# libxsmm/tpp-mlir

Hardware: AMD Instinct MI355X
Metric: GFLOP/s on BRGEMM 1024^3 fp32 br=16 (xsmm_brgemm_invoke) (higher is better)
Workload: dtype f32; 1 GPU; BRGEMM 1024x1024x1024 fp32, batch-reduce=16 (m=n=1024 k=64 lda=ldb=ldc=1024 stride_a=64 stride_b=65536 BETA_0), one independent problem per GPU; launch=invoke-loop, kernel=brgemm_f32_fast_lw<64x64,k2>

## Files before the change

tpp-mlir_amd/csrc/brgemm_f32_lw.hip:

```cpp
#include "brgemm_f32_lw_tile.h"
#include "chain_args.h"
#include "split_scratch.h"
#include <type_traits>

namespace tpp {

typedef __attribute__((address_space(1))) unsigned int g_u32_lw;

template <int WM, int WN, int WK, bool GROUPED, int NL = 1, int NSLOT = LW_NSLOT, int NLB = NL, bool SPLIT = false, bool TAIL = false>
__global__ __launch_bounds__(64 * (WM * WN * WK + NL + NLB)) void brgemm_f32_lw(GemmArgs p, const WorkItem *__restrict__ items) {
  static_assert(!TAIL || (!GROUPED && !SPLIT), "the tail split is an instance of its own");
  constexpr bool MAYSPLIT = SPLIT || TAIL;
  using Tile = LwTile<WM, WN, WK, NSLOT>;
  constexpr int NMW = Tile::NMW, BM = Tile::BM, BN = Tile::BN, IPG = Tile::IPG;

  const int tid = threadIdx.x, lane = tid & 63;
  const int hw_wave = __builtin_amdgcn_readfirstlane(tid >> 6);
  const int wave = hw_wave < NL + NLB ? NMW + hw_wave : hw_wave - (NL + NLB);
  static_assert(!SPLIT || WK > 1, "the split epilogue is the K-split tiles' float4 epilogue");
  constexpr bool RAGN = GROUPED || SPLIT;
  WorkItem it{p.A, p.B, p.C, p.D, (int64_t)p.br};
  int tm, tn, sp = 0, tile_id = 0;
  bool is_tail = false;
  if constexpr (TAIL) {
    const int per_block = p.tiles_m * p.tiles_n;
    const int xshift = (p.m / BM) * (p.n / BN) == per_block ? 0 : 3;
    const int body_per = p.tail_body >> xshift, tail_per = per_block - body_per;
    const int u = (int)blockIdx.x, x = u & ((1 << xshift) - 1);
    int lt = u >> xshift;
    is_tail = u >= p.tail_body;
    if (is_tail) {
      const int j = (u - p.tail_body) >> xshift, t = j % tail_per;
      sp = j / tail_per;
      tile_id = x * tail_per + t;
      lt = body_per + t;
    }
    const int tz = lt / p.tiles_n;
    tm = (x >> p.xn_shift) * p.tiles_m + tz;
    tn = (x & ((1 << p.xn_shift) - 1)) * p.tiles_n + (lt - tz * p.tiles_n);
  } else if constexpr (SPLIT && GROUPED) {
    const int item = (int)blockIdx.x / p.split;
    sp = (int)blockIdx.x - item * p.split;
    if (items) it = items[item];
    tm = (int)blockIdx.z, tn = (int)blockIdx.y;
    tile_id = (item * (int)gridDim.y + tn) * (int)gridDim.z + tm;
  } else if constexpr (SPLIT) {
    const int tiles = p.tiles_m * p.tiles_n, total = tiles * p.split;
    int u = (int)blockIdx.x;
    if ((total & 7) == 0) u = (u & 7) * (total >> 3) + (u >> 3);
    sp = u / tiles;
    tile_id = u - sp * tiles;
    tn = tile_id / p.tiles_m;
    tm = tile_id - tn * p.tiles_m;
  } else {
    if constexpr (GROUPED) {
      if (items) it = items[blockIdx.x];
    }
    tm = GROUPED ? (int)blockIdx.z : (int)(blockIdx.x >> p.xn_shift) * p.tiles_m + (int)blockIdx.z;
    tn = GROUPED ? (int)blockIdx.y : (int)(blockIdx.x & ((1u << p.xn_shift) - 1)) * p.tiles_n + (int)blockIdx.y;
  }
  const int m0 = tm * BM, n0 = tn * BN;
  const int nvalid = RAGN ? p.n - n0 : BN;
  const float *__restrict__ A = (const float *)it.A;
  const float *__restrict__ B = (const float *)it.B;
  float *__restrict__ C = (float *)it.C;
  const bool pair = GROUPED && p.k == 32;
  const int kchunks = pair ? 1 : p.k / LW_BK;
  const int Tall = pair ? (int)it.br / 2 : (int)it.br * kchunks;
  const int nsplit = TAIL && !is_tail ? 1 : p.split;
  const int t_first = MAYSPLIT ? (int)(((long long)Tall * sp) / nsplit) : 0;
  const int T = MAYSPLIT ? (int)(((long long)Tall * (sp + 1)) / nsplit) - t_first : Tall;

  if (wave >= NMW) {
    typename Tile::template Loader<NL, NLB> ld(wave - NMW, lane, A, B, m0, n0, (int)p.lda, (int)p.ldb, p.stride_a, p.stride_b, kchunks, pair, nvalid);
    if constexpr (MAYSPLIT) ld.start_at(t_first);
    lw_loader_schedule<NSLOT>(T, [&](int slot) __attribute__((always_inline)) { ld.issue(slot); },
                              [&](int chunks) __attribute__((always_inline)) { ld.wait_left(chunks); });
    return;
  }

  const typename Tile::Wave w(wave, lane);
  const int wk = w.wk, wm = w.wm, wn = w.wn;
  const int li = lane & 31, lh = lane >> 5;
  const int ccol = n0 + wn * 32 + li;
  const __amdgpu_buffer_rsrc_t rsrcC =
      __builtin_amdgcn_make_buffer_rsrc((void *)(C + (int64_t)m0 * p.ldc + n0), 0, 0x7fffffff, 0x00020000);
  const unsigned voffC = (unsigned)(((wm * 32 + 4 * lh) * (int)p.ldc + wn * 32 + li) * 4);
  const unsigned ldcb = (unsigned)((int)p.ldc * 4);
  f32x16 acc;
#pragma unroll
  for (int r = 0; r < 16; ++r) acc[r] = 0.0f;
  float bias = 0.0f;
  if constexpr (WK == 1) {
    if ((p.ep & EP_BIAS) && (!RAGN || ccol < p.n)) bias = ((const float *)it.D)[ccol];
  }
  constexpr bool BIAS_EARLY = WK > 1 && WM * WN * WK <= 4;
  f32x4 bias4 = {0.0f, 0.0f, 0.0f, 0.0f};
  const bool piece_ok = !RAGN || wn * 32 + 4 * (lane & 7) < nvalid;
  if constexpr (BIAS_EARLY) {
    if ((p.ep & EP_BIAS) && piece_ok) bias4 = *(const f32x4 *)((const float *)it.D + n0 + wn * 32 + 4 * (lane & 7));
  }
  if (wk == 0 && !SPLIT && !(TAIL && is_tail)) {
    if (!(p.ep & EP_BETA0) && (!RAGN || ccol < p.n)) {
#pragma unroll
      for (int r = 0; r < 16; ++r)
        acc[r] = __builtin_bit_cast(
            float, __builtin_amdgcn_raw_buffer_load_b32(rsrcC, voffC, (unsigned)((r & 3) + 8 * (r >> 2)) * ldcb, 0));
    }
  }

  __builtin_amdgcn_s_barrier();
  __builtin_amdgcn_sched_barrier(0);
  if (T > 0) Tile::mfma_chunks(acc, T, w);

  if constexpr (WK > 1) {
    Tile::park_partials(acc, w);
    if constexpr (!BIAS_EARLY) {
      if ((p.ep & EP_BIAS) && piece_ok) bias4 = *(const f32x4 *)((const float *)it.D + n0 + wn * 32 + 4 * (lane & 7));
    }
    f32x4 part[IPG];
    Tile::sum_partials(part, w);
    if (MAYSPLIT && (!TAIL || is_tail)) {
      constexpr int TILE = BM * BN;
      const int S = nsplit;
      float *scr = p.scratch + (size_t)tile_id * S * TILE;
      const __amdgpu_buffer_rsrc_t rsrcS = __builtin_amdgcn_make_buffer_rsrc((void *)scr, 0, 0x7fffffff, 0x00020000);
      const unsigned pvo = (unsigned)((wave * 64 + lane) * 16);
#pragma unroll
      for (int j = 0; j < IPG; ++j)
        __builtin_amdgcn_raw_buffer_store_b128(__builtin_bit_cast(u32x4, part[j]), rsrcS, pvo, (unsigned)((sp * TILE + j * NMW * 256) * 4), 16);
      asm volatile("s_waitcnt vmcnt(0)" ::: "memory");
      __syncthreads();
      unsigned *flag = (unsigned *)smem_lw;
      if (wave == 0 && lane == 0)
        *flag = __hip_atomic_fetch_add((g_u32_lw *)(p.split_cnt + tile_id), 1u, __ATOMIC_RELAXED, __HIP_MEMORY_SCOPE_AGENT);
      __syncthreads();
      if (*flag != (unsigned)(S - 1)) return;
      if (wave == 0 && lane == 0) __hip_atomic_store((g_u32_lw *)(p.split_cnt + tile_id), 0u, __ATOMIC_RELAXED, __HIP_MEMORY_SCOPE_AGENT);
#pragma unroll
      for (int j = 0; j < IPG; ++j) {
        f32x4 acc4 = __builtin_bit_cast(f32x4, __builtin_amdgcn_raw_buffer_load_b128(rsrcS, pvo, (unsigned)((j * NMW * 256) * 4), 16));
        int s2 = 1;
        for (; s2 + 4 <= S; s2 += 4) {
          f32x4 t[4];
#pragma unroll
          for (int e = 0; e < 4; ++e)
            t[e] = __builtin_bit_cast(f32x4, __builtin_amdgcn_raw_buffer_load_b128(rsrcS, pvo, (unsigned)(((s2 + e) * TILE + j * NMW * 256) * 4), 16));
#pragma unroll
          for (int e = 0; e < 4; ++e) acc4 += t[e];
        }
        for (; s2 < S; ++s2)
          acc4 += __builtin_bit_cast(f32x4, __builtin_amdgcn_raw_buffer_load_b128(rsrcS, pvo, (unsigned)((s2 * TILE + j * NMW * 256) * 4), 16));
        part[j] = acc4;
      }
#pragma unroll
      for (int j = 0; j < IPG; ++j) {
        if (!(p.ep & EP_BETA0) && piece_ok) part[j] += __builtin_bit_cast(f32x4, __builtin_amdgcn_raw_buffer_load_b128(rsrcC, Tile::piece_off(w, j, (int)p.ldc), 0, 0));
      }
    }
    Tile::finish(part, bias4, p.ep, rsrcC, (int)p.ldc, piece_ok, w);
    return;
  }
#pragma unroll
  for (int r = 0; r < 16; ++r) {
    float v = acc[r] + bias;
    if (p.ep & EP_RELU) v = v > 0.0f ? v : 0.0f;
    if (!RAGN || ccol < p.n)
      __builtin_amdgcn_raw_buffer_store_b32(__builtin_bit_cast(unsigned, v), rsrcC, voffC,
                                            (unsigned)((r & 3) + 8 * (r >> 2)) * ldcb, LW_C_AUX);
  }
}

typedef __attribute__((address_space(1))) unsigned int g_u32_f32c;
template <int WM, int WN, int WK, int NL>
__global__ __launch_bounds__(64 * (WM * WN * WK + 2 * NL)) void brgemm_f32_lw_chain(ChainArgs p) {
  static_assert(WK > 1, "the hand-off needs the 16-byte stores of the K-split tiles' epilogue");
  using Tile = LwTile<WM, WN, WK>;
  constexpr int NMW = Tile::NMW, BM = Tile::BM, BN = Tile::BN;

  const int tid = threadIdx.x, lane = tid & 63;
  const int hw_wave = __builtin_amdgcn_readfirstlane(tid >> 6);
  const int wave = hw_wave < 2 * NL ? NMW + hw_wave : hw_wave - 2 * NL;
  const int tm = (int)blockIdx.x / p.tiles_n, tn = (int)blockIdx.x % p.tiles_n;
  const int m0 = tm * BM, n0 = tn * BN;
  const int L = p.nlayers;

  if (wave >= NMW) {
    const bool isA = (wave - NMW) < NL;
    for (int l = 0; l < L; ++l) {
      const ChainLayer &Y = p.L[l];
      const int lda = (int)(l == 0 ? p.lda : p.L[l > 0 ? l - 1 : 0].ldc);
      const float *Asrc = (const float *)(l == 0 ? p.A : p.L[l > 0 ? l - 1 : 0].C);
      const int kchunks = Y.k / LW_BK;
      typename Tile::template Loader<NL, NL> ld(wave - NMW, lane, Asrc, (const float *)Y.B, m0, n0, lda, (int)Y.ldb, Y.stride_a, Y.stride_b, kchunks, false, BN);
      const bool sc1 = isA && l > 0;
      if (sc1) {
        g_u32_f32c *c = (g_u32_f32c *)(p.cnt + ((size_t)(l - 1) * p.tiles_m + tm) * CHAIN_CNT_STRIDE);
        const unsigned target = p.target;
        const unsigned long long t0 = __builtin_amdgcn_s_memrealtime();
        for (;;) {
          const unsigned v = __hip_atomic_load(c, __ATOMIC_RELAXED, __HIP_MEMORY_SCOPE_AGENT);
          if ((int)(v - target) >= 0) break;
          if (__builtin_amdgcn_s_memrealtime() - t0 > CHAIN_TIMEOUT_TICKS) {
            if (lane == 0) __hip_atomic_store((g_u32_f32c *)p.err, 1u + (unsigned)l, __ATOMIC_RELAXED, __HIP_MEMORY_SCOPE_AGENT);
            break;
          }
          __builtin_amdgcn_s_sleep(1);
        }
        asm volatile("" ::: "memory");
      }
      lw_loader_schedule<LW_NSLOT>(Y.br * kchunks, [&](int slot) __attribute__((always_inline)) { ld.template issue<true>(slot, sc1); },
                                   [&](int chunks) __attribute__((always_inline)) { ld.wait_left(chunks); });
      __builtin_amdgcn_s_barrier();
      __builtin_amdgcn_s_barrier();
      if (l + 1 < L) __builtin_amdgcn_s_barrier();
    }
    return;
  }

  const typename Tile::Wave w(wave, lane);
  for (int l = 0; l < L; ++l) {
    const ChainLayer &Y = p.L[l];
    const int ldc = (int)Y.ldc;
    const __amdgpu_buffer_rsrc_t rsrcC = __builtin_amdgcn_make_buffer_rsrc((void *)((float *)Y.C + (int64_t)m0 * ldc + n0), 0, 0x7fffffff, 0x00020000);
    f32x16 acc;
#pragma unroll
    for (int r = 0; r < 16; ++r) acc[r] = 0.0f;
    __builtin_amdgcn_s_barrier();
    __builtin_amdgcn_sched_barrier(0);
    Tile::mfma_chunks(acc, Y.br * (Y.k / LW_BK), w);
    Tile::park_partials(acc, w);
    f32x4 bias4 = {0.0f, 0.0f, 0.0f, 0.0f}, part[Tile::IPG];
    if (Y.ep & EP_BIAS) bias4 = *(const f32x4 *)((const float *)Y.D + n0 + w.wn * 32 + 4 * (lane & 7));
    Tile::sum_partials(part, w);
    Tile::finish(part, bias4, Y.ep, rsrcC, ldc, true, w);
    if (l + 1 == L) break;
    asm volatile("s_waitcnt vmcnt(0) lgkmcnt(0)" ::: "memory");
    __builtin_amdgcn_s_barrier();
    if (wave == 0 && lane == 0)
      __hip_atomic_fetch_add((g_u32_f32c *)(p.cnt + ((size_t)l * p.tiles_m + tm) * CHAIN_CNT_STRIDE), 1u, __ATOMIC_RELAXED, __HIP_MEMORY_SCOPE_AGENT);
  }
}

template <int WM, int WN, int WK, int NL, int NSLOT, int NLB>
__global__ __launch_bounds__(64 * (WM * WN * WK + NL + NLB)) void brgemm_f32_lw_edge(GemmArgs p) {
  using Tile = LwTile<WM, WN, WK, NSLOT>;
  constexpr int NMW = Tile::NMW, BM = Tile::BM, BN = Tile::BN, IPG = Tile::IPG;

  const int tid = threadIdx.x, lane = tid & 63;
  const int hw_wave = __builtin_amdgcn_readfirstlane(tid >> 6);
  const int wave = hw_wave < NL + NLB ? NMW + hw_wave : hw_wave - (NL + NLB);
  const int tm = (int)(blockIdx.x >> p.xn_shift) * p.tiles_m + (int)blockIdx.z;
  const int tn = (int)(blockIdx.x & ((1u << p.xn_shift) - 1)) * p.tiles_n + (int)blockIdx.y;
  const int m0 = tm * BM < p.m - BM ? tm * BM : p.m - BM, n0 = tn * BN < p.n - BN ? tn * BN : p.n - BN;
  const int own_r = tm * BM - m0, own_c = tn * BN - n0;
  const float *__restrict__ A = (const float *)p.A;
  const float *__restrict__ B = (const float *)p.B;
  float *__restrict__ C = (float *)p.C;
  const int kchunks = p.k / LW_BK;
  const int T = p.br * kchunks;

  if (wave >= NMW) {
    typename Tile::template Loader<NL, NLB> ld(wave - NMW, lane, A, B, m0, n0, (int)p.lda, (int)p.ldb, p.stride_a, p.stride_b, kchunks, false, BN);
    lw_loader_schedule<NSLOT>(T, [&](int slot) __attribute__((always_inline)) { ld.issue(slot); },
                              [&](int chunks) __attribute__((always_inline)) { ld.wait_left(chunks); });
    return;
  }

  const typename Tile::Wave w(wave, lane);
  const int wk = w.wk, wm = w.wm, wn = w.wn;
  const int li = lane & 31, lh = lane >> 5;
  const __amdgpu_buffer_rsrc_t rsrcC =
      __builtin_amdgcn_make_buffer_rsrc((void *)(C + (int64_t)m0 * p.ldc + n0), 0, 0x7fffffff, 0x00020000);
  const unsigned voffC = (unsigned)(((wm * 32 + 4 * lh) * (int)p.ldc + wn * 32 + li) * 4);
  const unsigned ldcb = (unsigned)((int)p.ldc * 4);
  const bool col_owned = wn * 32 + li >= own_c;
  const int row_first = own_r - (wm * 32 + 4 * lh);
  f32x16 acc;
#pragma unroll
  for (int r = 0; r < 16; ++r) acc[r] = 0.0f;
  float bias = 0.0f;
  if constexpr (WK == 1) {
    if (p.ep & EP_BIAS) bias = ((const float *)p.D)[n0 + wn * 32 + li];
  }
  constexpr bool BIAS_EARLY = WK > 1 && WM * WN * WK <= 4;
  f32x4 bias4 = {0.0f, 0.0f, 0.0f, 0.0f};
  if constexpr (BIAS_EARLY) {
    if (p.ep & EP_BIAS) bias4 = *(const f32x4 *)((const float *)p.D + n0 + wn * 32 + 4 * (lane & 7));
  }
  if (wk == 0 && !(p.ep & EP_BETA0) && col_owned) {
#pragma unroll
    for (int r = 0; r < 16; ++r)
      if ((r & 3) + 8 * (r >> 2) >= row_first)
        acc[r] = __builtin_bit_cast(float, __builtin_amdgcn_raw_buffer_load_b32(rsrcC, voffC, (unsigned)((r & 3) + 8 * (r >> 2)) * ldcb, 0));
  }

  __builtin_amdgcn_s_barrier();
  __builtin_amdgcn_sched_barrier(0);
  if (T > 0) Tile::mfma_chunks(acc, T, w);

  if constexpr (WK > 1) {
    Tile::park_partials(acc, w);
    if constexpr (!BIAS_EARLY) {
      if (p.ep & EP_BIAS) bias4 = *(const f32x4 *)((const float *)p.D + n0 + wn * 32 + 4 * (lane & 7));
    }
    f32x4 part[IPG];
    Tile::sum_partials(part, w);
    Tile::finish_owned(part, bias4, p.ep, rsrcC, (int)p.ldc, own_r, own_c, w);
    return;
  }
#pragma unroll
  for (int r = 0; r < 16; ++r) {
    float v = acc[r] + bias;
    if (p.ep & EP_RELU) v = v > 0.0f ? v : 0.0f;
    if (col_owned && (r & 3) + 8 * (r >> 2) >= row_first)
      __builtin_amdgcn_raw_buffer_store_b32(__builtin_bit_cast(unsigned, v), rsrcC, voffC, (unsigned)((r & 3) + 8 * (r >> 2)) * ldcb, LW_C_AUX);
  }
}

template <int WM, int WN, int WK, int NL, int NSLOT, int NLB>
__global__ __launch_bounds__(64 * (WM * WN * WK + NL + NLB)) void brgemm_f32_lw_kedge(GemmArgs p) {
  using Tile = LwTile<WM, WN, WK, NSLOT>;
  constexpr int NMW = Tile::NMW, BM = Tile::BM, BN = Tile::BN, IPG = Tile::IPG;

  const int tid = threadIdx.x, lane = tid & 63;
  const int hw_wave = __builtin_amdgcn_readfirstlane(tid >> 6);
  const int wave = hw_wave < NL + NLB ? NMW + hw_wave : hw_wave - (NL + NLB);
  const int tm = (int)(blockIdx.x >> p.xn_shift) * p.tiles_m + (int)blockIdx.z;
  const int tn = (int)(blockIdx.x & ((1u << p.xn_shift) - 1)) * p.tiles_n + (int)blockIdx.y;
  const int m0 = tm * BM < p.m - BM ? tm * BM : p.m - BM, n0 = tn * BN < p.n - BN ? tn * BN : p.n - BN;
  const int own_r = tm * BM - m0, own_c = tn * BN - n0;
  const float *__restrict__ A = (const float *)p.A;
  const float *__restrict__ B = (const float *)p.B;
  float *__restrict__ C = (float *)p.C;
  const int kchunks = kedge_chunks(p.k);
  const int T = p.br * kchunks;

  if (wave >= NMW) {
    typename Tile::template Loader<NL, NLB> ld(wave - NMW, lane, A, B, m0, n0, (int)p.lda, (int)p.ldb, p.stride_a, p.stride_b, kchunks, false, BN);
    ld.ragged_k(p.k);
    lw_loader_schedule<NSLOT>(T, [&](int slot) __attribute__((always_inline)) { ld.issue_ragged(slot); },
                              [&](int chunks) __attribute__((always_inline)) { ld.wait_left(chunks); });
    return;
  }

  const typename Tile::Wave w(wave, lane);
  const int wk = w.wk, wm = w.wm, wn = w.wn;
  const int li = lane & 31, lh = lane >> 5;
  const __amdgpu_buffer_rsrc_t rsrcC =
      __builtin_amdgcn_make_buffer_rsrc((void *)(C + (int64_t)m0 * p.ldc + n0), 0, 0x7fffffff, 0x00020000);
  const unsigned voffC = (unsigned)(((wm * 32 + 4 * lh) * (int)p.ldc + wn * 32 + li) * 4);
  const unsigned ldcb = (unsigned)((int)p.ldc * 4);
  const bool col_owned = wn * 32 + li >= own_c;
  const int row_first = own_r - (wm * 32 + 4 * lh);
  f32x16 acc;
#pragma unroll
  for (int r = 0; r < 16; ++r) acc[r] = 0.0f;
  float bias = 0.0f;
  if constexpr (WK == 1) {
    if (p.ep & EP_BIAS) bias = ((const float *)p.D)[n0 + wn * 32 + li];
  }
  constexpr bool BIAS_EARLY = WK > 1 && WM * WN * WK <= 4;
  f32x4 bias4 = {0.0f, 0.0f, 0.0f, 0.0f};
  if constexpr (BIAS_EARLY) {
    if (p.ep & EP_BIAS) bias4 = *(const f32x4 *)((const float *)p.D + n0 + wn * 32 + 4 * (lane & 7));
  }
  if (wk == 0 && !(p.ep & EP_BETA0) && col_owned) {
#pragma unroll
    for (int r = 0; r < 16; ++r)
      if ((r & 3) + 8 * (r >> 2) >= row_first)
        acc[r] = __builtin_bit_cast(float, __builtin_amdgcn_raw_buffer_load_b32(rsrcC, voffC, (unsigned)((r & 3) + 8 * (r >> 2)) * ldcb, 0));
  }

  __builtin_amdgcn_s_barrier();
  __builtin_amdgcn_sched_barrier(0);
  Tile::mfma_chunks_ragged(acc, T, kchunks, kedge_skip_blocks(p.k, kchunks - 1), w);

  if constexpr (WK > 1) {
    Tile::park_partials(acc, w);
    if constexpr (!BIAS_EARLY) {
      if (p.ep & EP_BIAS) bias4 = *(const f32x4 *)((const float *)p.D + n0 + wn * 32 + 4 * (lane & 7));
    }
    f32x4 part[IPG];
    Tile::sum_partials(part, w);
    Tile::finish_owned(part, bias4, p.ep, rsrcC, (int)p.ldc, own_r, own_c, w);
    return;
  }
#pragma unroll
  for (int r = 0; r < 16; ++r) {
    float v = acc[r] + bias;
    if (p.ep & EP_RELU) v = v > 0.0f ? v : 0.0f;
    if (col_owned && (r & 3) + 8 * (r >> 2) >= row_first)
      __builtin_amdgcn_raw_buffer_store_b32(__builtin_bit_cast(unsigned, v), rsrcC, voffC, (unsigned)((r & 3) + 8 * (r >> 2)) * ldcb, LW_C_AUX);
  }
}

static int lw_xcd_blocks(const GemmArgs &a, int tiles_m, int tiles_n) {
  int xm = 0;
  long long best = -1;
  for (int c : {4, 2, 8, 1}) {
    const int xn = 8 / c;
    if (tiles_m % c || tiles_n % xn || tiles_m / c > 65535 || tiles_n / xn > 65535) continue;
    const long long cost = (long long)a.m / c + (long long)a.n / xn;
    if (best < 0 || cost < best) {
      best = cost;
      xm = c;
    }
  }
  return xm;
}

static bool lw_xcd_grid(GemmArgs &args, int tiles_m, int tiles_n, bool allow_blocks = true) {
  const int xm = allow_blocks ? lw_xcd_blocks(args, tiles_m, tiles_n) : 0, xn = xm ? 8 / xm : 1;
  args.tiles_m = xm ? tiles_m / xm : tiles_m;
  args.tiles_n = tiles_n / xn;
  args.xn_shift = xn == 8 ? 3 : xn == 4 ? 2 : xn == 2 ? 1 : 0;
  return xm != 0;
}

static bool lw_split_scratch(GemmArgs &args, hipStream_t s, long long tiles, int S, int tile_floats) {
  const SplitScratch *sc = split_scratch_for(s, tiles, tiles * S * tile_floats);
  if (!sc) return false;
  args.split = S;
  args.scratch = sc->partial;
  args.split_cnt = sc->cnt;
  return true;
}

template <int WM, int WN, int WK, bool GROUPED = false, int NL = 1, int NSLOT = LW_NSLOT, int NLB = NL, bool SPLIT = false, bool TAIL = false> struct LwLayer {
  using Tile = LwTile<WM, WN, WK, NSLOT>;
  static constexpr int NT = 64 * (Tile::NMW + NL + NLB);
  static constexpr auto kernel = brgemm_f32_lw<WM, WN, WK, GROUPED, NL, NSLOT, NLB, SPLIT, TAIL>;
};
template <int WM, int WN, int WK, int NL> struct LwChain {
  using Tile = LwTile<WM, WN, WK>;
  static constexpr int NT = 64 * (Tile::NMW + 2 * NL);
  static constexpr auto kernel = brgemm_f32_lw_chain<WM, WN, WK, NL>;
};
template <int WM, int WN, int WK, int NL, int NSLOT, int NLB> struct LwEdge {
  using Tile = LwTile<WM, WN, WK, NSLOT>;
  static constexpr int NT = 64 * (Tile::NMW + NL + NLB);
  static constexpr auto kernel = brgemm_f32_lw_edge<WM, WN, WK, NL, NSLOT, NLB>;
};
template <int WM, int WN, int WK, int NL, int NSLOT, int NLB> struct LwKEdge {
  using Tile = LwTile<WM, WN, WK, NSLOT>;
  static constexpr int NT = 64 * (Tile::NMW + NL + NLB);
  static constexpr auto kernel = brgemm_f32_lw_kedge<WM, WN, WK, NL, NSLOT, NLB>;
};
template <class I, class... Args> static hipError_t lw_launch(dim3 grid, hipStream_t s, const Args &...args) {
  static std::atomic<unsigned long long> lds_set{0};
  if (hipError_t e = ensure_dynamic_lds((const void *)I::kernel, (int)I::Tile::LDS_BYTES, lds_set); e != hipSuccess) return e;
  hipLaunchKernelGGL(I::kernel, grid, dim3(I::NT), I::Tile::LDS_BYTES, s, args...);
  return hipGetLastError();
}

template <int WM, int WN, int WK, int NL = 1, int NSLOT = LW_NSLOT, int NLB = NL> static hipError_t launch_lw_t(const GemmArgs &a, hipStream_t s) {
  using I = LwLayer<WM, WN, WK, false, NL, NSLOT, NLB>;
  GemmArgs args = a;
  const bool blocks = lw_xcd_grid(args, a.m / I::Tile::BM, a.n / I::Tile::BN);
  if (args.tiles_m > 65535 || args.tiles_n > 65535) return hipErrorInvalidValue;
  return lw_launch<I>(dim3(blocks ? 8 : 1, args.tiles_n, args.tiles_m), s, args, (const WorkItem *)nullptr);
}

template <int WM, int WN, int WK, bool SPLIT>
static hipError_t launch_lw_grouped_t(const GemmArgs &a, const WorkItem *items, int n_items, int S, hipStream_t s) {
  using I = LwLayer<WM, WN, WK, true, 1, LW_NSLOT, 1, SPLIT>;
  constexpr int BM = I::Tile::BM, BN = I::Tile::BN;
  const int tiles_m = a.m / BM, tiles_n = (a.n + BN - 1) / BN;
  GemmArgs args = a;
  args.tiles_m = args.tiles_n = 0;
  args.xn_shift = 0;
  if (SPLIT && !lw_split_scratch(args, s, (long long)n_items * tiles_m * tiles_n, S, BM * BN)) return hipErrorOutOfMemory;
  return lw_launch<I>(dim3((unsigned)(n_items * (SPLIT ? S : 1)), tiles_n, tiles_m), s, args, items);
}

template <int WM, int WN, int WK> static hipError_t launch_lw_split_t(const GemmArgs &a, int S, hipStream_t s) {
  using I = LwLayer<WM, WN, WK, false, 1, LW_NSLOT, 1, true>;
  constexpr int BM = I::Tile::BM, BN = I::Tile::BN;
  GemmArgs args = a;
  args.tiles_m = a.m / BM;
  args.tiles_n = (a.n + BN - 1) / BN;
  args.xn_shift = 0;
  const long long tiles = (long long)args.tiles_m * args.tiles_n;
  if (!lw_split_scratch(args, s, tiles, S, BM * BN)) return hipErrorOutOfMemory;
  return lw_launch<I>(dim3((unsigned)(tiles * S)), s, args, (const WorkItem *)nullptr);
}
template <int WM, int WN, int WK, int NL, int NLB> static hipError_t launch_lw_tail_t(const GemmArgs &a, int tail_tiles, int S, hipStream_t s) {
  using I = LwLayer<WM, WN, WK, false, NL, LW_NSLOT, NLB, false, true>;
  constexpr int BM = I::Tile::BM, BN = I::Tile::BN;
  const int tiles_m = a.m / BM, tiles_n = a.n / BN;
  const long long tiles = (long long)tiles_m * tiles_n, body = tiles - tail_tiles;
  if (a.m % BM || a.n % BN || tail_tiles <= 0 || body <= 0 || S < 2 || S > SPLIT_MAX || body + (long long)tail_tiles * S > 0x7fffffffLL)
    return hipErrorInvalidValue;
  GemmArgs args = a;
  if (!lw_split_scratch(args, s, tail_tiles, S, BM * BN)) return hipErrorOutOfMemory;
  lw_xcd_grid(args, tiles_m, tiles_n, body % 8 == 0 && tail_tiles % 8 == 0);
  args.tail_body = (int)body;
  return lw_launch<I>(dim3((unsigned)(body + (long long)tail_tiles * S)), s, args, (const WorkItem *)nullptr);
}

template <int WM, int WN, int WK, int NL = 1, int NSLOT = LW_NSLOT, int NLB = NL> static hipError_t launch_lw_edge_t(const GemmArgs &a, hipStream_t s) {
  using I = LwEdge<WM, WN, WK, NL, NSLOT, NLB>;
  constexpr int BM = I::Tile::BM, BN = I::Tile::BN;
  if (a.m < BM || a.n < BN || (a.n & 3) || a.k <= 0 || a.k % LW_BK || a.br < 1) return hipErrorInvalidValue;
  GemmArgs args = a;
  const bool blocks = lw_xcd_grid(args, (a.m + BM - 1) / BM, (a.n + BN - 1) / BN);
  if (args.tiles_m > 65535 || args.tiles_n > 65535) return hipErrorInvalidValue;
  return lw_launch<I>(dim3(blocks ? 8 : 1, args.tiles_n, args.tiles_m), s, args);
}

template <int WM, int WN, int WK, int NL = 1, int NSLOT = LW_NSLOT, int NLB = NL> static hipError_t launch_lw_kedge_t(const GemmArgs &a, hipStream_t s) {
  using I = LwKEdge<WM, WN, WK, NL, NSLOT, NLB>;
  constexpr int BM = I::Tile::BM, BN = I::Tile::BN;
  if (a.m < BM || a.n < BN || (a.n & 3) || !kedge_k_ok(a.k) || a.br < 1) return hipErrorInvalidValue;
  GemmArgs args = a;
  const bool blocks = lw_xcd_grid(args, (a.m + BM - 1) / BM, (a.n + BN - 1) / BN);
  if (args.tiles_m > 65535 || args.tiles_n > 65535) return hipErrorInvalidValue;
  return lw_launch<I>(dim3(blocks ? 8 : 1, args.tiles_n, args.tiles_m), s, args);
}

hipError_t launch_f32_lw_halves(const GemmArgs &a, hipStream_t s) {
  if (a.m <= 0 || a.n <= 0 || a.m % 64 || a.n % 64 || a.k <= 0 || a.k % LW_BK || a.br < 0) return hipErrorInvalidValue;
  return launch_lw_t<2, 1, 2, 2, 3, 1>(a, s);
}

hipError_t launch_f32_lw_grouped(int tile, const GemmArgs &a, const WorkItem *items, int n_items, int split, hipStream_t s) {
  if (split > 1) {
    hipError_t e = hipErrorInvalidValue;
    switch (tile) {
    case 1: e = launch_lw_grouped_t<2, 2, 2, true>(a, items, n_items, split, s); break;
    case 2: e = launch_lw_grouped_t<2, 1, 4, true>(a, items, n_items, split, s); break;
    case 3: e = launch_lw_grouped_t<1, 1, 4, true>(a, items, n_items, split, s); break;
    default: break;
    }
    if (e != hipErrorOutOfMemory && e != hipErrorInvalidValue) return e;
    (void)hipGetLastError();
  }
  switch (tile) {
  case 0: return launch_lw_grouped_t<2, 2, 1, false>(a, items, n_items, 1, s);
  case 1: return launch_lw_grouped_t<2, 2, 2, false>(a, items, n_items, 1, s);
  case 2: return launch_lw_grouped_t<2, 1, 4, false>(a, items, n_items, 1, s);
  case 3: return launch_lw_grouped_t<1, 1, 4, false>(a, items, n_items, 1, s);
  default: return hipErrorInvalidValue;
  }
}
hipError_t launch_f32_lw_split(int tile, const GemmArgs &a, int split, hipStream_t s) {
  switch (tile) {
  case 1: return launch_lw_split_t<2, 2, 2>(a, split, s);
  case 2: return launch_lw_split_t<2, 1, 4>(a, split, s);
  case 3: return launch_lw_split_t<1, 1, 4>(a, split, s);
  default: return hipErrorInvalidValue;
  }
}

hipError_t launch_f32_lw_tail(int tile, const GemmArgs &a, int tail_tiles, int split, hipStream_t s) {
  switch (tile) {
  case 1: return launch_lw_tail_t<2, 2, 2, 2, 2>(a, tail_tiles, split, s);
  case 2: return launch_lw_tail_t<2, 1, 4, 2, 1>(a, tail_tiles, split, s);
  case 3: return launch_lw_tail_t<1, 1, 4, 1, 1>(a, tail_tiles, split, s);
  default: return hipErrorInvalidValue;
  }
}

hipError_t launch_f32_lw_edge(int tile, const GemmArgs &a, hipStream_t s) {
  switch (tile) {
  case 1: return launch_lw_edge_t<2, 2, 2, 2>(a, s);
  case 2: return launch_lw_edge_t<2, 1, 4, 2, LW_NSLOT, 1>(a, s);
  case 3: return launch_lw_edge_t<1, 1, 4>(a, s);
  case 4: return launch_lw_edge_t<4, 2, 1, 2, 3>(a, s);
  default: return hipErrorInvalidValue;
  }
}

hipError_t launch_f32_lw_kedge(int tile, const GemmArgs &a, hipStream_t s) {
  switch (tile) {
  case 1: return launch_lw_kedge_t<2, 2, 2, 2>(a, s);
  case 2: return launch_lw_kedge_t<2, 1, 4, 2, LW_NSLOT, 1>(a, s);
  case 3: return launch_lw_kedge_t<1, 1, 4>(a, s);
  case 4: return launch_lw_kedge_t<4, 2, 1, 2, 3>(a, s);
  default: return hipErrorInvalidValue;
  }
}

template <int WM, int WN, int WK, int NL> static hipError_t launch_f32_chain_t(const ChainArgs &a, hipStream_t s) {
  using I = LwChain<WM, WN, WK, NL>;
  ChainArgs args = a;
  args.tiles_m = a.m / I::Tile::BM;
  args.tiles_n = a.n / I::Tile::BN;
  const long long tiles = (long long)args.tiles_m * args.tiles_n;
  if (tiles <= 0 || tiles > 0x7fffffffLL) return hipErrorInvalidValue;
  return lw_launch<I>(dim3((unsigned)tiles), s, args);
}

hipError_t launch_f32_chain(int tile, const ChainArgs &a, hipStream_t s) {
  switch (tile) {
  case 1: return launch_f32_chain_t<2, 2, 2, 2>(a, s);
  case 2: return launch_f32_chain_t<2, 1, 4, 1>(a, s);
  default: return hipErrorInvalidValue;
  }
}

hipError_t launch_f32_lw(int tile, const GemmArgs &a, hipStream_t s) {
  switch (tile) {
  case 0: return launch_lw_t<2, 2, 1>(a, s);
  case 1: return launch_lw_t<2, 2, 2, 2>(a, s);
  case 2: return launch_lw_t<2, 1, 4, 2, LW_NSLOT, 1>(a, s);
  case 3: return launch_lw_t<1, 1, 4>(a, s);
  case 4: return launch_lw_t<4, 2, 1, 2, 3>(a, s);
  default: return hipErrorInvalidValue;
  }
}

}
```

tpp-mlir_amd/csrc/brgemm_f32_lw_tile.h:

```cpp
#pragma once
#include "brgemm_f32_lw_kedge.h"
#include "gemm_common.h"
#include "xsmm_desc.h"
#include <type_traits>

namespace tpp {

constexpr int LW_BK = 64;
constexpr int LW_NSLOT = 4;
constexpr int LW_C_AUX = C_STORE_AUX;
static_assert(KEDGE_BK == LW_BK, "the ragged-k schedule is written for this chunk");

typedef __attribute__((address_space(3))) void lds_void_lw;
extern __shared__ __attribute__((aligned(16))) float smem_lw[];

template <int NSLOT, class Issue, class Wait> __device__ __forceinline__ void lw_loader_schedule(int T, Issue &&issue, Wait &&wait_left) {
  if (T > 0) issue(0);
  if (T > 1) issue(1);
  wait_left(T > 1 ? 1 : 0);
  __builtin_amdgcn_s_barrier();
  if (NSLOT > 3 && T > 2) issue(2);
  for (int t = 0; t + 1 < T; ++t) {
    wait_left(NSLOT > 3 && t + 2 < T ? 1 : 0);
    __builtin_amdgcn_s_barrier();
    if (t + NSLOT - 1 < T) issue((t + NSLOT - 1) % NSLOT);
  }
}

template <int WM, int WN, int WK, int NSLOT = LW_NSLOT> struct LwTile {
  static constexpr int NMW = WM * WN * WK;
  static constexpr int BM = 32 * WM, BN = 32 * WN;
  static constexpr int A_STAGE = BM * LW_BK, B_STAGE = LW_BK * BN, SLOT = A_STAGE + B_STAGE;
  static constexpr int NA = BM / 4;
  static constexpr int RPI = 256 / BN;
  static constexpr int NB = LW_BK / RPI;
  static constexpr int KB_PER_WAVE = 8 / WK, KB_HALF = KB_PER_WAVE / 2;
  static constexpr int IPG = WK > 1 ? 4 / WK : 1;
  static constexpr size_t LDS_BYTES = (size_t)NSLOT * SLOT * sizeof(float);
  static_assert(KB_HALF >= 1, "tile outside the schedule's limits");
  static_assert(NSLOT == 3 || NSLOT == 4, "ring depth");
  static_assert(LDS_BYTES <= 160 * 1024, "LDS budget");

  template <int NL, int NLB> struct Loader {
    static_assert(NA % NL == 0 && NB % NLB == 0, "panel instructions divide over the loader waves");
    static_assert(NA / NL <= 31 && NB / NLB <= 31, "tile outside the schedule's limits (vmcnt is 6 bits)");
    bool isA;
    int part, kc, kchunks;
    unsigned voA[4], voA2[2], voB, stepA, stepB, pairB;
    const float *g;
    int64_t d_in, d_batch, d_wrap;

    __device__ __forceinline__ Loader(int lw, int lane, const float *A, const float *B, int m0, int n0, int lda, int ldb, int64_t stride_a,
                                      int64_t stride_b, int kchunks_, bool pair, int nvalid)
        : isA(lw < NL), part(lw < NL ? lw : lw - NL), kc(0), kchunks(kchunks_) {
#pragma unroll
      for (int j = 0; j < 4; ++j) {
        const int r = 4 * j + (lane >> 4), pc = (lane & 15) ^ r;
        voA[j] = (unsigned)((r * lda + (pair ? (pc >> 3) * (int)stride_a + 4 * (pc & 7) : 4 * pc)) * 4);
      }
#pragma unroll
      for (int j = 0; j < 2; ++j) {
        const int r = 4 * (part + 2 * j) + (lane >> 4), pc = (lane & 15) ^ r;
        voA2[j] = (unsigned)((r * lda + (pair ? (pc >> 3) * (int)stride_a + 4 * (pc & 7) : 4 * pc)) * 4);
      }
      const int pieceB = nvalid < BN ? (lane % (BN / 4) < nvalid / 4 ? lane % (BN / 4) : nvalid / 4 - 1) : lane % (BN / 4);
      voB = (unsigned)(((lane / (BN / 4)) * ldb + 4 * pieceB) * 4);
      stepA = (unsigned)(16 * lda * 4), stepB = (unsigned)(RPI * ldb * 4);
      pairB = pair ? (unsigned)(((int)stride_b - 32 * ldb) * 4) : 0u;
      g = isA ? A + (int64_t)m0 * lda : B + n0;
      d_in = isA ? (int64_t)LW_BK : (int64_t)LW_BK * ldb;
      d_batch = (isA ? stride_a : stride_b) * (pair ? 2 : 1);
      d_wrap = d_batch - (int64_t)(kchunks - 1) * d_in;
    }
    __device__ __forceinline__ void start_at(int t_first) {
      const int b0 = t_first / kchunks;
      kc = t_first - b0 * kchunks;
      g += (int64_t)b0 * d_batch + (int64_t)kc * d_in;
    }
    template <int AUX> __device__ __forceinline__ void load_a(float *base, __amdgpu_buffer_rsrc_t r) const {
#pragma unroll
      for (int i = 0; i < NA / NL; ++i) {
        const int v = part + NL * i;
        __builtin_amdgcn_raw_ptr_buffer_load_lds(r, (lds_void_lw *)(base + v * 256), 16, NL == 1 ? voA[i & 3] : NL == 2 ? voA2[i & 1] : voA2[0],
                                                 (unsigned)(v >> 2) * stepA, 0, AUX);
      }
    }
    template <bool MAY_SC1 = false> __device__ __forceinline__ void issue(int slot, bool sc1 = false) {
      float *base = smem_lw + slot * SLOT + (isA ? 0 : A_STAGE);
      const __amdgpu_buffer_rsrc_t r = __builtin_amdgcn_make_buffer_rsrc((void *)g, 0, 0x7fffffff, 0x00020000);
      if (isA) {
        if (MAY_SC1 && sc1) load_a<16>(base, r);
        else load_a<0>(base, r);
      } else {
#pragma unroll
        for (int i = 0; i < NB / NLB; ++i) {
          const int v = part + NLB * i;
          __builtin_amdgcn_raw_ptr_buffer_load_lds(r, (lds_void_lw *)(base + v * 256), 16, voB, (unsigned)v * stepB + (v * RPI >= 32 ? pairB : 0u), 0, 0);
        }
      }
      if (++kc == kchunks) {
        kc = 0;
        g += d_wrap;
      } else {
        g += d_in;
      }
    }
    int64_t d_fix;
    __device__ __forceinline__ void ragged_k(int k) {
      const int64_t unit = d_in / LW_BK;
      d_fix = (int64_t)(kedge_step(k, kchunks - 2) - LW_BK) * unit;
      d_wrap = d_batch - (int64_t)kedge_chunk_start(k, kchunks - 1) * unit;
    }
    __device__ __forceinline__ void issue_ragged(int slot) {
      issue(slot);
      if (kc == kchunks - 1) g += d_fix;
    }
    __device__ __forceinline__ void wait_left(int chunks) const {
      if (chunks == 0) asm volatile("s_waitcnt vmcnt(0)" ::: "memory");
      else if (isA) asm volatile("s_waitcnt vmcnt(%0)" ::"n"(NA / NL) : "memory");
      else asm volatile("s_waitcnt vmcnt(%0)" ::"n"(NB / NLB) : "memory");
    }
  };

  struct Wave {
    int wk, wmn, wm, wn, lane;
    __device__ __forceinline__ Wave(int wave, int lane_) : wk(wave / (WM * WN)), wmn(wave % (WM * WN)), wm(wmn / WN), wn(wmn % WN), lane(lane_) {}
  };

  static __device__ __forceinline__ void mfma_chunks(f32x16 &acc, int T, const Wave &w) {
    f32x4 fa[2];
    float fb[2][4];
    const int li = w.lane & 31, lh = w.lane >> 5;
    const int a_off = (w.wm * 32 + li) * LW_BK, b_off = w.wn * 32 + li;
    auto frag_load = [&](int buf, int slot, int kb) __attribute__((always_inline)) {
      const float *as = smem_lw + slot * SLOT + a_off;
      const float *bs = smem_lw + slot * SLOT + A_STAGE + b_off;
      fa[buf] = *(const f32x4 *)(as + (((2 * kb + lh) ^ (li & 15)) << 2));
#pragma unroll
      for (int s = 0; s < 4; ++s) fb[buf][s] = bs[(8 * kb + 4 * lh + s) * BN];
    };
    const int kbw = w.wk * KB_PER_WAVE;
    auto chunk = [&](auto slot_c, auto hn_c, bool has_next_rt) __attribute__((always_inline)) {
      constexpr int S = decltype(slot_c)::value, NS = (S + 1) % NSLOT;
      const bool has_next = decltype(hn_c)::value == 1 ? true : has_next_rt;
#pragma unroll
      for (int q = 0; q < KB_PER_WAVE; ++q) {
        const int cur = q & 1, nxt = cur ^ 1;
        if (q + 1 < KB_PER_WAVE) frag_load(nxt, S, kbw + q + 1);
        else frag_load(nxt, NS, kbw);
        __builtin_amdgcn_sched_barrier(0);
#pragma unroll
        for (int s = 0; s < 4; ++s) acc = __builtin_amdgcn_mfma_f32_32x32x2f32(fa[cur][s], fb[cur][s], acc, 0, 0, 0);
        __builtin_amdgcn_sched_barrier(0);
        if (q == KB_HALF - 1 && has_next) {
          __builtin_amdgcn_s_barrier();
          __builtin_amdgcn_sched_barrier(0);
        }
      }
      constexpr int PF = KB_PER_WAVE & 1;
      if constexpr (decltype(hn_c)::value != 1)
        asm volatile("" : "+v"(fa[PF]), "+v"(fb[PF][0]), "+v"(fb[PF][1]), "+v"(fb[PF][2]), "+v"(fb[PF][3]));
    };
    using S0 = std::integral_constant<int, 0>;
    using S1 = std::integral_constant<int, 1>;
    using S2 = std::integral_constant<int, 2>;
    using S3 = std::integral_constant<int, 3>;
    using HY = std::integral_constant<int, 1>;
    using HR = std::integral_constant<int, 2>;

    frag_load(0, 0, kbw);
    int t = 0;
    for (; t + NSLOT < T; t += NSLOT) {
      chunk(S0{}, HY{}, true);
      chunk(S1{}, HY{}, true);
      chunk(S2{}, HY{}, true);
      if constexpr (NSLOT > 3) chunk(S3{}, HY{}, true);
    }
    for (;;) {
      chunk(S0{}, HR{}, t + 1 < T);
      if (++t == T) break;
      chunk(S1{}, HR{}, t + 1 < T);
      if (++t == T) break;
      chunk(S2{}, HR{}, t + 1 < T);
      if (++t == T) break;
      if constexpr (NSLOT > 3) {
        chunk(S3{}, HR{}, t + 1 < T);
        if (++t == T) break;
      }
    }
  }

  static __device__ __forceinline__ void mfma_chunks_ragged(f32x16 &acc, int T, int kchunks, int skip, const Wave &w) {
    f32x4 fa[2];
    float fb[2][4];
    const int li = w.lane & 31, lh = w.lane >> 5;
    const int a_off = (w.wm * 32 + li) * LW_BK, b_off = w.wn * 32 + li;
    auto frag_load = [&](int buf, int slot, int kb) __attribute__((always_inline)) {
      const float *as = smem_lw + slot * SLOT + a_off;
      const float *bs = smem_lw + slot * SLOT + A_STAGE + b_off;
      fa[buf] = *(const f32x4 *)(as + (((2 * kb + lh) ^ (li & 15)) << 2));
#pragma unroll
      for (int s = 0; s < 4; ++s) fb[buf][s] = bs[(8 * kb + 4 * lh + s) * BN];
    };
    const int kbw = w.wk * KB_PER_WAVE;
    auto chunk = [&](auto slot_c, auto rag_c, int first, bool has_next_rt) __attribute__((always_inline)) {
      constexpr int S = decltype(slot_c)::value, NS = (S + 1) % NSLOT;
      constexpr bool RAG = decltype(rag_c)::value != 0;
      const bool has_next = RAG ? has_next_rt : true;
#pragma unroll
      for (int q = 0; q < KB_PER_WAVE; ++q) {
        const int cur = q & 1, nxt = cur ^ 1;
        if (q + 1 < KB_PER_WAVE) frag_load(nxt, S, kbw + q + 1);
        else frag_load(nxt, NS, kbw);
        __builtin_amdgcn_sched_barrier(0);
        if (!RAG || kedge_block_runs(kbw + q, first)) {
#pragma unroll
          for (int s = 0; s < 4; ++s) acc = __builtin_amdgcn_mfma_f32_32x32x2f32(fa[cur][s], fb[cur][s], acc, 0, 0, 0);
        }
        __builtin_amdgcn_sched_barrier(0);
        if (q == KB_HALF - 1 && has_next) {
          __builtin_amdgcn_s_barrier();
          __builtin_amdgcn_sched_barrier(0);
        }
      }
      constexpr int PF = KB_PER_WAVE & 1;
      if constexpr (RAG) asm volatile("" : "+v"(fa[PF]), "+v"(fb[PF][0]), "+v"(fb[PF][1]), "+v"(fb[PF][2]), "+v"(fb[PF][3]));
    };
    using S0 = std::integral_constant<int, 0>;
    using S1 = std::integral_constant<int, 1>;
    using S2 = std::integral_constant<int, 2>;
    using S3 = std::integral_constant<int, 3>;
    using R0 = std::integral_constant<int, 0>;
    using R1 = std::integral_constant<int, 1>;

    frag_load(0, 0, kbw);
    int t = 0, c = 0;
    for (;;) {
      if (c + NSLOT < kchunks) {
        chunk(S0{}, R0{}, 0, true);
        chunk(S1{}, R0{}, 0, true);
        chunk(S2{}, R0{}, 0, true);
        if constexpr (NSLOT > 3) chunk(S3{}, R0{}, 0, true);
        t += NSLOT, c += NSLOT;
        continue;
      }
      chunk(S0{}, R1{}, c + 1 == kchunks ? skip : 0, t + 1 < T);
      if (++t == T) break;
      if (++c == kchunks) c = 0;
      chunk(S1{}, R1{}, c + 1 == kchunks ? skip : 0, t + 1 < T);
      if (++t == T) break;
      if (++c == kchunks) c = 0;
      chunk(S2{}, R1{}, c + 1 == kchunks ? skip : 0, t + 1 < T);
      if (++t == T) break;
      if (++c == kchunks) c = 0;
      if constexpr (NSLOT > 3) {
        chunk(S3{}, R1{}, c + 1 == kchunks ? skip : 0, t + 1 < T);
        if (++t == T) break;
        if (++c == kchunks) c = 0;
      }
    }
  }

  static __device__ __forceinline__ void park_partials(const f32x16 &acc, const Wave &w) {
    __syncthreads();
    float *dst = smem_lw + (w.wk * (WM * WN) + w.wmn) * 1024 + w.lane;
#pragma unroll
    for (int r = 0; r < 16; ++r) dst[r * 64] = acc[r];
    __syncthreads();
  }
  static __device__ __forceinline__ int piece_row(const Wave &w, int j) { return 8 * (w.wk * IPG + j) + (w.lane >> 3); }
  static __device__ __forceinline__ unsigned piece_off(const Wave &w, int j, int ldc) {
    return (unsigned)(((w.wm * 32 + piece_row(w, j)) * ldc + w.wn * 32 + 4 * (w.lane & 7)) * 4);
  }
  static __device__ __forceinline__ void sum_partials(f32x4 (&part)[IPG], const Wave &w) {
#pragma unroll
    for (int j = 0; j < IPG; ++j) {
      const int q = piece_row(w, j);
      const int r = (q & 3) + 4 * (q >> 3), lh2 = (q >> 2) & 1;
      const float *src = smem_lw + w.wmn * 1024 + r * 64 + lh2 * 32 + 4 * (w.lane & 7);
      f32x4 v = *(const f32x4 *)src;
#pragma unroll
      for (int g = 1; g < WK; ++g) v += *(const f32x4 *)(src + g * (WM * WN) * 1024);
      part[j] = v;
    }
  }
  static __device__ __forceinline__ void finish(const f32x4 (&part)[IPG], f32x4 bias4, int ep, __amdgpu_buffer_rsrc_t rsrcC, int ldc, bool ok, const Wave &w) {
#pragma unroll
    for (int j = 0; j < IPG; ++j) {
      f32x4 v = part[j] + bias4;
      if (ep & EP_RELU) {
#pragma unroll
        for (int e = 0; e < 4; ++e) v[e] = v[e] > 0.0f ? v[e] : 0.0f;
      }
      if (ok) __builtin_amdgcn_raw_buffer_store_b128(__builtin_bit_cast(u32x4, v), rsrcC, piece_off(w, j, ldc), 0, LW_C_AUX);
    }
  }
  static __device__ __forceinline__ bool piece_owned(const Wave &w, int j, int own_r, int own_c) {
    return w.wm * 32 + piece_row(w, j) >= own_r && w.wn * 32 + 4 * (w.lane & 7) >= own_c;
  }
  static __device__ __forceinline__ void finish_owned(const f32x4 (&part)[IPG], f32x4 bias4, int ep, __amdgpu_buffer_rsrc_t rsrcC, int ldc, int own_r, int own_c,
                                                      const Wave &w) {
#pragma unroll
    for (int j = 0; j < IPG; ++j) {
      f32x4 v = part[j] + bias4;
      if (ep & EP_RELU) {
#pragma unroll
        for (int e = 0; e < 4; ++e) v[e] = v[e] > 0.0f ? v[e] : 0.0f;
      }
      if (piece_owned(w, j, own_r, own_c)) __builtin_amdgcn_raw_buffer_store_b128(__builtin_bit_cast(u32x4, v), rsrcC, piece_off(w, j, ldc), 0, LW_C_AUX);
    }
  }
};

}
```

Before: 123,900 GFLOP/s.

## Precompute and pin LDS fragment and epilogue addresses; overlap loader setup with first load

Computes LDS fragment addresses, park/sum addresses and C store offsets once before the main loop and pins them in registers with empty asm constraints. This removes per-chunk address arithmetic from the MFMA loop. The loader now issues the first chunk's load before computing the batch/wrap strides, so setup work overlaps the first memory request. Kernel arguments are forced into scalar registers. The cost is higher VGPR pressure from holding the precomputed addresses, which could lower occupancy or cause spills.

Result: faster. 127,400 GFLOP/s, median of 6 (+2.8%).

```diff
diff --git a/tpp-mlir_amd/csrc/brgemm_f32_lw.hip b/tpp-mlir_amd/csrc/brgemm_f32_lw.hip
--- a/tpp-mlir_amd/csrc/brgemm_f32_lw.hip
+++ b/tpp-mlir_amd/csrc/brgemm_f32_lw.hip
@@ -61,8 +61,12 @@
   }
   const int m0 = tm * BM, n0 = tn * BN;
   const int nvalid = RAGN ? p.n - n0 : BN;
-  const float *__restrict__ A = (const float *)it.A;
-  const float *__restrict__ B = (const float *)it.B;
+  const float *A_ = (const float *)it.A, *B_ = (const float *)it.B;
+  int lda = (int)p.lda, ldb = (int)p.ldb;
+  int64_t stride_a = p.stride_a, stride_b = p.stride_b;
+  asm volatile("" : "+s"(A_), "+s"(B_), "+s"(lda), "+s"(ldb), "+s"(stride_a), "+s"(stride_b));
+  const float *__restrict__ A = A_;
+  const float *__restrict__ B = B_;
   float *__restrict__ C = (float *)it.C;
   const bool pair = GROUPED && p.k == 32;
   const int kchunks = pair ? 1 : p.k / LW_BK;
@@ -72,10 +76,17 @@
   const int T = MAYSPLIT ? (int)(((long long)Tall * (sp + 1)) / nsplit) - t_first : Tall;
 
   if (wave >= NMW) {
-    typename Tile::template Loader<NL, NLB> ld(wave - NMW, lane, A, B, m0, n0, (int)p.lda, (int)p.ldb, p.stride_a, p.stride_b, kchunks, pair, nvalid);
-    if constexpr (MAYSPLIT) ld.start_at(t_first);
+    typename Tile::template Loader<NL, NLB> ld(wave - NMW, lane, A, B, m0, n0, lda, ldb, stride_a, stride_b, kchunks, pair, nvalid);
+    if constexpr (MAYSPLIT) {
+      ld.finish_setup();
+      ld.start_at(t_first);
+    }
     lw_loader_schedule<NSLOT>(T, [&](int slot) __attribute__((always_inline)) { ld.issue(slot); },
-                              [&](int chunks) __attribute__((always_inline)) { ld.wait_left(chunks); });
+                              [&](int chunks) __attribute__((always_inline)) { ld.wait_left(chunks); },
+                              [&]() __attribute__((always_inline)) {
+                                if constexpr (MAYSPLIT) ld.issue(0);
+                                else ld.issue_first();
+                              });
     return;
   }
 
@@ -109,17 +120,21 @@
     }
   }
 
+  const auto fr = Tile::mfma_setup(w);
+  const auto tl = Tile::template tail_setup<!SPLIT>(w, (int)p.ldc);
+  const int Tp = Tile::pin_chunks(T);
+
   __builtin_amdgcn_s_barrier();
   __builtin_amdgcn_sched_barrier(0);
-  if (T > 0) Tile::mfma_chunks(acc, T, w);
+  if (Tp > 0) Tile::mfma_chunks(acc, Tp, fr);
 
   if constexpr (WK > 1) {
-    Tile::park_partials(acc, w);
+    Tile::park_partials(acc, tl);
     if constexpr (!BIAS_EARLY) {
       if ((p.ep & EP_BIAS) && piece_ok) bias4 = *(const f32x4 *)((const float *)it.D + n0 + wn * 32 + 4 * (lane & 7));
     }
     f32x4 part[IPG];
-    Tile::sum_partials(part, w);
+    Tile::sum_partials(part, tl);
     if (MAYSPLIT && (!TAIL || is_tail)) {
       constexpr int TILE = BM * BN;
       const int S = nsplit;
@@ -155,10 +170,10 @@
       }
 #pragma unroll
       for (int j = 0; j < IPG; ++j) {
-        if (!(p.ep & EP_BETA0) && piece_ok) part[j] += __builtin_bit_cast(f32x4, __builtin_amdgcn_raw_buffer_load_b128(rsrcC, Tile::piece_off(w, j, (int)p.ldc), 0, 0));
+        if (!(p.ep & EP_BETA0) && piece_ok) part[j] += __builtin_bit_cast(f32x4, __builtin_amdgcn_raw_buffer_load_b128(rsrcC, Tile::tail_off(tl, j), 0, 0));
       }
     }
-    Tile::finish(part, bias4, p.ep, rsrcC, (int)p.ldc, piece_ok, w);
+    Tile::finish(part, bias4, p.ep, rsrcC, piece_ok, tl);
     return;
   }
 #pragma unroll
@@ -210,7 +225,8 @@
         asm volatile("" ::: "memory");
       }
       lw_loader_schedule<LW_NSLOT>(Y.br * kchunks, [&](int slot) __attribute__((always_inline)) { ld.template issue<true>(slot, sc1); },
-                                   [&](int chunks) __attribute__((always_inline)) { ld.wait_left(chunks); });
+                                   [&](int chunks) __attribute__((always_inline)) { ld.wait_left(chunks); },
+                                   [&]() __attribute__((always_inline)) { ld.template issue_first<true>(sc1); });
       __builtin_amdgcn_s_barrier();
       __builtin_amdgcn_s_barrier();
       if (l + 1 < L) __builtin_amdgcn_s_barrier();
@@ -219,6 +235,8 @@
   }
 
   const typename Tile::Wave w(wave, lane);
+  constexpr bool CHAIN_PIN = !(WM == 2 && WN == 2);
+  const auto fr = Tile::template mfma_setup<CHAIN_PIN>(w);
   for (int l = 0; l < L; ++l) {
     const ChainLayer &Y = p.L[l];
     const int ldc = (int)Y.ldc;
@@ -226,14 +244,16 @@
     f32x16 acc;
 #pragma unroll
     for (int r = 0; r < 16; ++r) acc[r] = 0.0f;
+    const auto tl = Tile::template tail_setup<CHAIN_PIN>(w, ldc);
+    const int T = Tile::template pin_chunks<CHAIN_PIN>(Y.br * (Y.k / LW_BK));
     __builtin_amdgcn_s_barrier();
     __builtin_amdgcn_sched_barrier(0);
-    Tile::mfma_chunks(acc, Y.br * (Y.k / LW_BK), w);
-    Tile::park_partials(acc, w);
+    Tile::mfma_chunks(acc, T, fr);
+    Tile::park_partials(acc, tl);
     f32x4 bias4 = {0.0f, 0.0f, 0.0f, 0.0f}, part[Tile::IPG];
     if (Y.ep & EP_BIAS) bias4 = *(const f32x4 *)((const float *)Y.D + n0 + w.wn * 32 + 4 * (lane & 7));
-    Tile::sum_partials(part, w);
-    Tile::finish(part, bias4, Y.ep, rsrcC, ldc, true, w);
+    Tile::sum_partials(part, tl);
+    Tile::finish(part, bias4, Y.ep, rsrcC, true, tl);
     if (l + 1 == L) break;
     asm volatile("s_waitcnt vmcnt(0) lgkmcnt(0)" ::: "memory");
     __builtin_amdgcn_s_barrier();
@@ -254,16 +274,21 @@
   const int tn = (int)(blockIdx.x & ((1u << p.xn_shift) - 1)) * p.tiles_n + (int)blockIdx.y;
   const int m0 = tm * BM < p.m - BM ? tm * BM : p.m - BM, n0 = tn * BN < p.n - BN ? tn * BN : p.n - BN;
   const int own_r = tm * BM - m0, own_c = tn * BN - n0;
-  const float *__restrict__ A = (const float *)p.A;
-  const float *__restrict__ B = (const float *)p.B;
+  const float *A_ = (const float *)p.A, *B_ = (const float *)p.B;
+  int lda = (int)p.lda, ldb = (int)p.ldb;
+  int64_t stride_a = p.stride_a, stride_b = p.stride_b;
+  asm volatile("" : "+s"(A_), "+s"(B_), "+s"(lda), "+s"(ldb), "+s"(stride_a), "+s"(stride_b));
+  const float *__restrict__ A = A_;
+  const float *__restrict__ B = B_;
   float *__restrict__ C = (float *)p.C;
   const int kchunks = p.k / LW_BK;
   const int T = p.br * kchunks;
 
   if (wave >= NMW) {
-    typename Tile::template Loader<NL, NLB> ld(wave - NMW, lane, A, B, m0, n0, (int)p.lda, (int)p.ldb, p.stride_a, p.stride_b, kchunks, false, BN);
+    typename Tile::template Loader<NL, NLB> ld(wave - NMW, lane, A, B, m0, n0, lda, ldb, stride_a, stride_b, kchunks, false, BN);
     lw_loader_schedule<NSLOT>(T, [&](int slot) __attribute__((always_inline)) { ld.issue(slot); },
-                              [&](int chunks) __attribute__((always_inline)) { ld.wait_left(chunks); });
+                              [&](int chunks) __attribute__((always_inline)) { ld.wait_left(chunks); },
+                              [&]() __attribute__((always_inline)) { ld.issue_first(); });
     return;
   }
 
@@ -295,18 +320,22 @@
         acc[r] = __builtin_bit_cast(float, __builtin_amdgcn_raw_buffer_load_b32(rsrcC, voffC, (unsigned)((r & 3) + 8 * (r >> 2)) * ldcb, 0));
   }
 
+  const auto fr = Tile::mfma_setup(w);
+  const auto tl = Tile::tail_setup(w, (int)p.ldc);
+  const int Tp = Tile::pin_chunks(T);
+
   __builtin_amdgcn_s_barrier();
   __builtin_amdgcn_sched_barrier(0);
-  if (T > 0) Tile::mfma_chunks(acc, T, w);
+  if (Tp > 0) Tile::mfma_chunks(acc, Tp, fr);
 
   if constexpr (WK > 1) {
-    Tile::park_partials(acc, w);
+    Tile::park_partials(acc, tl);
     if constexpr (!BIAS_EARLY) {
       if (p.ep & EP_BIAS) bias4 = *(const f32x4 *)((const float *)p.D + n0 + wn * 32 + 4 * (lane & 7));
     }
     f32x4 part[IPG];
-    Tile::sum_partials(part, w);
-    Tile::finish_owned(part, bias4, p.ep, rsrcC, (int)p.ldc, own_r, own_c, w);
+    Tile::sum_partials(part, tl);
+    Tile::finish_owned(part, bias4, p.ep, rsrcC, own_r, own_c, w, tl);
     return;
   }
 #pragma unroll
@@ -330,17 +359,21 @@
   const int tn = (int)(blockIdx.x & ((1u << p.xn_shift) - 1)) * p.tiles_n + (int)blockIdx.y;
   const int m0 = tm * BM < p.m - BM ? tm * BM : p.m - BM, n0 = tn * BN < p.n - BN ? tn * BN : p.n - BN;
   const int own_r = tm * BM - m0, own_c = tn * BN - n0;
-  const float *__restrict__ A = (const float *)p.A;
-  const float *__restrict__ B = (const float *)p.B;
+  const float *A_ = (const float *)p.A, *B_ = (const float *)p.B;
+  int lda = (int)p.lda, ldb = (int)p.ldb;
+  int64_t stride_a = p.stride_a, stride_b = p.stride_b;
+  asm volatile("" : "+s"(A_), "+s"(B_), "+s"(lda), "+s"(ldb), "+s"(stride_a), "+s"(stride_b));
+  const float *__restrict__ A = A_;
+  const float *__restrict__ B = B_;
   float *__restrict__ C = (float *)p.C;
   const int kchunks = kedge_chunks(p.k);
   const int T = p.br * kchunks;
 
   if (wave >= NMW) {
-    typename Tile::template Loader<NL, NLB> ld(wave - NMW, lane, A, B, m0, n0, (int)p.lda, (int)p.ldb, p.stride_a, p.stride_b, kchunks, false, BN);
-    ld.ragged_k(p.k);
+    typename Tile::template Loader<NL, NLB> ld(wave - NMW, lane, A, B, m0, n0, lda, ldb, stride_a, stride_b, kchunks, false, BN);
     lw_loader_schedule<NSLOT>(T, [&](int slot) __attribute__((always_inline)) { ld.issue_ragged(slot); },
-                              [&](int chunks) __attribute__((always_inline)) { ld.wait_left(chunks); });
+                              [&](int chunks) __attribute__((always_inline)) { ld.wait_left(chunks); },
+                              [&]() __attribute__((always_inline)) { ld.issue_first_ragged(p.k); });
     return;
   }
 
@@ -372,18 +405,22 @@
         acc[r] = __builtin_bit_cast(float, __builtin_amdgcn_raw_buffer_load_b32(rsrcC, voffC, (unsigned)((r & 3) + 8 * (r >> 2)) * ldcb, 0));
   }
 
+  const auto fr = Tile::template mfma_setup<false>(w);
+  const auto tl = Tile::template tail_setup<false>(w, (int)p.ldc);
+  const int Tp = T;
+
   __builtin_amdgcn_s_barrier();
   __builtin_amdgcn_sched_barrier(0);
-  Tile::mfma_chunks_ragged(acc, T, kchunks, kedge_skip_blocks(p.k, kchunks - 1), w);
+  Tile::mfma_chunks_ragged(acc, Tp, kchunks, kedge_skip_blocks(p.k, kchunks - 1), fr);
 
   if constexpr (WK > 1) {
-    Tile::park_partials(acc, w);
+    Tile::park_partials(acc, tl);
     if constexpr (!BIAS_EARLY) {
       if (p.ep & EP_BIAS) bias4 = *(const f32x4 *)((const float *)p.D + n0 + wn * 32 + 4 * (lane & 7));
     }
     f32x4 part[IPG];
-    Tile::sum_partials(part, w);
-    Tile::finish_owned(part, bias4, p.ep, rsrcC, (int)p.ldc, own_r, own_c, w);
+    Tile::sum_partials(part, tl);
+    Tile::finish_owned(part, bias4, p.ep, rsrcC, own_r, own_c, w, tl);
     return;
   }
 #pragma unroll
diff --git a/tpp-mlir_amd/csrc/brgemm_f32_lw_tile.h b/tpp-mlir_amd/csrc/brgemm_f32_lw_tile.h
--- a/tpp-mlir_amd/csrc/brgemm_f32_lw_tile.h
+++ b/tpp-mlir_amd/csrc/brgemm_f32_lw_tile.h
@@ -14,8 +14,9 @@
 typedef __attribute__((address_space(3))) void lds_void_lw;
 extern __shared__ __attribute__((aligned(16))) float smem_lw[];
 
-template <int NSLOT, class Issue, class Wait> __device__ __forceinline__ void lw_loader_schedule(int T, Issue &&issue, Wait &&wait_left) {
-  if (T > 0) issue(0);
+template <int NSLOT, class Issue, class Wait, class First>
+__device__ __forceinline__ void lw_loader_schedule(int T, Issue &&issue, Wait &&wait_left, First &&first) {
+  if (T > 0) first();
   if (T > 1) issue(1);
   wait_left(T > 1 ? 1 : 0);
   __builtin_amdgcn_s_barrier();
@@ -26,6 +27,16 @@
     if (t + NSLOT - 1 < T) issue((t + NSLOT - 1) % NSLOT);
   }
 }
+
+template <int NSLOT, class Issue, class Wait> __device__ __forceinline__ void lw_loader_schedule(int T, Issue &&issue, Wait &&wait_left) {
+  lw_loader_schedule<NSLOT>(T, issue, wait_left, [&]() __attribute__((always_inline)) { issue(0); });
+}
+
+typedef __attribute__((address_space(3))) float lds_float_lw;
+typedef __attribute__((address_space(3))) f32x4 lds_f32x4_lw;
+__device__ __forceinline__ unsigned lw_lds_addr(const float *p) { return (unsigned)(__SIZE_TYPE__)(const lds_float_lw *)p; }
+__device__ __forceinline__ lds_float_lw *lw_lds_float(unsigned a) { return (lds_float_lw *)(__SIZE_TYPE__)a; }
+__device__ __forceinline__ const lds_f32x4_lw *lw_lds_f32x4(unsigned a) { return (const lds_f32x4_lw *)(__SIZE_TYPE__)a; }
 
 template <int WM, int WN, int WK, int NSLOT = LW_NSLOT> struct LwTile {
   static constexpr int NMW = WM * WN * WK;
@@ -54,23 +65,39 @@
                                       int64_t stride_b, int kchunks_, bool pair, int nvalid)
         : isA(lw < NL), part(lw < NL ? lw : lw - NL), kc(0), kchunks(kchunks_) {
 #pragma unroll
-      for (int j = 0; j < 4; ++j) {
-        const int r = 4 * j + (lane >> 4), pc = (lane & 15) ^ r;
-        voA[j] = (unsigned)((r * lda + (pair ? (pc >> 3) * (int)stride_a + 4 * (pc & 7) : 4 * pc)) * 4);
-      }
-#pragma unroll
-      for (int j = 0; j < 2; ++j) {
-        const int r = 4 * (part + 2 * j) + (lane >> 4), pc = (lane & 15) ^ r;
-        voA2[j] = (unsigned)((r * lda + (pair ? (pc >> 3) * (int)stride_a + 4 * (pc & 7) : 4 * pc)) * 4);
-      }
-      const int pieceB = nvalid < BN ? (lane % (BN / 4) < nvalid / 4 ? lane % (BN / 4) : nvalid / 4 - 1) : lane % (BN / 4);
-      voB = (unsigned)(((lane / (BN / 4)) * ldb + 4 * pieceB) * 4);
-      stepA = (unsigned)(16 * lda * 4), stepB = (unsigned)(RPI * ldb * 4);
-      pairB = pair ? (unsigned)(((int)stride_b - 32 * ldb) * 4) : 0u;
-      g = isA ? A + (int64_t)m0 * lda : B + n0;
-      d_in = isA ? (int64_t)LW_BK : (int64_t)LW_BK * ldb;
-      d_batch = (isA ? stride_a : stride_b) * (pair ? 2 : 1);
-      d_wrap = d_batch - (int64_t)(kchunks - 1) * d_in;
+      for (int j = 0; j < 4; ++j) voA[j] = 0u;
+      voA2[0] = voA2[1] = voB = stepA = stepB = pairB = 0u;
+      if (isA) {
+        g = A + (int64_t)m0 * lda;
+#pragma unroll
+        for (int j = 0; j < 4; ++j) {
+          const int r = 4 * j + (lane >> 4), pc = (lane & 15) ^ r;
+          voA[j] = (unsigned)((r * lda + (pair ? (pc >> 3) * (int)stride_a + 4 * (pc & 7) : 4 * pc)) * 4);
+        }
+#pragma unroll
+        for (int j = 0; j < 2; ++j) {
+          const int r = 4 * (part + 2 * j) + (lane >> 4), pc = (lane & 15) ^ r;
+          voA2[j] = (unsigned)((r * lda + (pair ? (pc >> 3) * (int)stride_a + 4 * (pc & 7) : 4 * pc)) * 4);
+        }
+        stepA = (unsigned)(16 * lda * 4);
+      } else {
+        g = B + n0;
+        const int pieceB = nvalid < BN ? (lane % (BN / 4) < nvalid / 4 ? lane % (BN / 4) : nvalid / 4 - 1) : lane % (BN / 4);
+        voB = (unsigned)(((lane / (BN / 4)) * ldb + 4 * pieceB) * 4);
+        stepB = (unsigned)(RPI * ldb * 4);
+        pairB = pair ? (unsigned)(((int)stride_b - 32 * ldb) * 4) : 0u;
+      }
+      ldb_ = ldb, stride_a_ = stride_a, stride_b_ = stride_b, pair_ = pair;
+    }
+    int ldb_;
+    int64_t stride_a_, stride_b_;
+    bool pair_;
+    __device__ __forceinline__ void finish_setup() {
+      int kch = kchunks;
+      asm volatile("" : "+s"(kch));
+      d_in = isA ? (int64_t)LW_BK : (int64_t)LW_BK * ldb_;
+      d_batch = (isA ? stride_a_ : stride_b_) * (pair_ ? 2 : 1);
+      d_wrap = d_batch - (int64_t)(kch - 1) * d_in;
     }
     __device__ __forceinline__ void start_at(int t_first) {
       const int b0 = t_first / kchunks;
@@ -86,6 +113,15 @@
       }
     }
     template <bool MAY_SC1 = false> __device__ __forceinline__ void issue(int slot, bool sc1 = false) {
+      request<MAY_SC1>(slot, sc1);
+      advance();
+    }
+    template <bool MAY_SC1 = false> __device__ __forceinline__ void issue_first(bool sc1 = false) {
+      request<MAY_SC1>(0, sc1);
+      finish_setup();
+      advance();
+    }
+    template <bool MAY_SC1> __device__ __forceinline__ void request(int slot, bool sc1) const {
       float *base = smem_lw + slot * SLOT + (isA ? 0 : A_STAGE);
       const __amdgpu_buffer_rsrc_t r = __builtin_amdgcn_make_buffer_rsrc((void *)g, 0, 0x7fffffff, 0x00020000);
       if (isA) {
@@ -98,6 +134,8 @@
           __builtin_amdgcn_raw_ptr_buffer_load_lds(r, (lds_void_lw *)(base + v * 256), 16, voB, (unsigned)v * stepB + (v * RPI >= 32 ? pairB : 0u), 0, 0);
         }
       }
+    }
+    __device__ __forceinline__ void advance() {
       if (++kc == kchunks) {
         kc = 0;
         g += d_wrap;
@@ -115,6 +153,13 @@
       issue(slot);
       if (kc == kchunks - 1) g += d_fix;
     }
+    __device__ __forceinline__ void issue_first_ragged(int k) {
+      request<false>(0, false);
+      finish_setup();
+      ragged_k(k);
+      advance();
+      if (kc == kchunks - 1) g += d_fix;
+    }
     __device__ __forceinline__ void wait_left(int chunks) const {
       if (chunks == 0) asm volatile("s_waitcnt vmcnt(0)" ::: "memory");
       else if (isA) asm volatile("s_waitcnt vmcnt(%0)" ::"n"(NA / NL) : "memory");
@@ -127,27 +172,68 @@
     __device__ __forceinline__ Wave(int wave, int lane_) : wk(wave / (WM * WN)), wmn(wave % (WM * WN)), wm(wmn / WN), wn(wmn % WN), lane(lane_) {}
   };
 
-  static __device__ __forceinline__ void mfma_chunks(f32x16 &acc, int T, const Wave &w) {
+  static constexpr int A_SPG = (65535 - 15) / (SLOT * 4) + 1, A_GRP = (NSLOT + A_SPG - 1) / A_SPG;
+  static constexpr bool PIN_DEFAULT = WK > 1;
+  template <bool PIN> struct Frags {
+    unsigned a[PIN ? A_GRP : 1][KB_PER_WAVE], b[PIN ? NSLOT : 1][KB_PER_WAVE];
+    int kbw;
+    int li, lh, a_off, b_off;
+    __device__ __forceinline__ void load(f32x4 &fa, float (&fb)[4], int slot, int q) const {
+      if constexpr (PIN) {
+        fa = *lw_lds_f32x4(a[slot / A_SPG][q] + (unsigned)((slot % A_SPG) * SLOT * 4));
+        const lds_float_lw *bs = lw_lds_float(b[slot][q]);
+#pragma unroll
+        for (int s = 0; s < 4; ++s) fb[s] = bs[s * BN];
+      } else {
+        const int kb = kbw + q;
+        const float *as = smem_lw + slot * SLOT + a_off;
+        const float *bs = smem_lw + slot * SLOT + A_STAGE + b_off;
+        fa = *(const f32x4 *)(as + (((2 * kb + lh) ^ (li & 15)) << 2));
+#pragma unroll
+        for (int s = 0; s < 4; ++s) fb[s] = bs[(8 * kb + 4 * lh + s) * BN];
+      }
+    }
+  };
+  template <bool PIN = PIN_DEFAULT> static __device__ __forceinline__ Frags<PIN> mfma_setup(const Wave &w) {
+    Frags<PIN> f = {};
+    f.li = w.lane & 31, f.lh = w.lane >> 5;
+    f.a_off = (w.wm * 32 + f.li) * LW_BK, f.b_off = w.wn * 32 + f.li;
+    f.kbw = w.wk * KB_PER_WAVE;
+    if constexpr (PIN) {
+#pragma unroll
+      for (int q = 0; q < KB_PER_WAVE; ++q) {
+        const int kb = f.kbw + q;
+#pragma unroll
+        for (int g = 0; g < A_GRP; ++g) {
+          f.a[g][q] = lw_lds_addr(smem_lw + g * A_SPG * SLOT + f.a_off + (((2 * kb + f.lh) ^ (f.li & 15)) << 2));
+          asm volatile("" : "+v"(f.a[g][q]));
+        }
+#pragma unroll
+        for (int slot = 0; slot < NSLOT; ++slot) {
+          f.b[slot][q] = lw_lds_addr(smem_lw + slot * SLOT + A_STAGE + f.b_off + (8 * kb + 4 * f.lh) * BN);
+          asm volatile("" : "+v"(f.b[slot][q]));
+        }
+      }
+    }
+    return f;
+  }
+  template <bool PIN = PIN_DEFAULT> static __device__ __forceinline__ int pin_chunks(int T) {
+    if constexpr (PIN) asm volatile("" : "+s"(T));
+    return T;
+  }
+
+  template <bool PIN> static __device__ __forceinline__ void mfma_chunks(f32x16 &acc, int T, const Frags<PIN> &f) {
     f32x4 fa[2];
     float fb[2][4];
-    const int li = w.lane & 31, lh = w.lane >> 5;
-    const int a_off = (w.wm * 32 + li) * LW_BK, b_off = w.wn * 32 + li;
-    auto frag_load = [&](int buf, int slot, int kb) __attribute__((always_inline)) {
-      const float *as = smem_lw + slot * SLOT + a_off;
-      const float *bs = smem_lw + slot * SLOT + A_STAGE + b_off;
-      fa[buf] = *(const f32x4 *)(as + (((2 * kb + lh) ^ (li & 15)) << 2));
-#pragma unroll
-      for (int s = 0; s < 4; ++s) fb[buf][s] = bs[(8 * kb + 4 * lh + s) * BN];
-    };
-    const int kbw = w.wk * KB_PER_WAVE;
+    auto frag_load = [&](int buf, int slot, int q) __attribute__((always_inline)) { f.load(fa[buf], fb[buf], slot, q); };
     auto chunk = [&](auto slot_c, auto hn_c, bool has_next_rt) __attribute__((always_inline)) {
       constexpr int S = decltype(slot_c)::value, NS = (S + 1) % NSLOT;
       const bool has_next = decltype(hn_c)::value == 1 ? true : has_next_rt;
 #pragma unroll
       for (int q = 0; q < KB_PER_WAVE; ++q) {
         const int cur = q & 1, nxt = cur ^ 1;
-        if (q + 1 < KB_PER_WAVE) frag_load(nxt, S, kbw + q + 1);
-        else frag_load(nxt, NS, kbw);
+        if (q + 1 < KB_PER_WAVE) frag_load(nxt, S, q + 1);
+        else frag_load(nxt, NS, 0);
         __builtin_amdgcn_sched_barrier(0);
 #pragma unroll
         for (int s = 0; s < 4; ++s) acc = __builtin_amdgcn_mfma_f32_32x32x2f32(fa[cur][s], fb[cur][s], acc, 0, 0, 0);
@@ -168,7 +254,7 @@
     using HY = std::integral_constant<int, 1>;
     using HR = std::integral_constant<int, 2>;
 
-    frag_load(0, 0, kbw);
+    frag_load(0, 0, 0);
     int t = 0;
     for (; t + NSLOT < T; t += NSLOT) {
       chunk(S0{}, HY{}, true);
@@ -190,19 +276,11 @@
     }
   }
 
-  static __device__ __forceinline__ void mfma_chunks_ragged(f32x16 &acc, int T, int kchunks, int skip, const Wave &w) {
+  template <bool PIN> static __device__ __forceinline__ void mfma_chunks_ragged(f32x16 &acc, int T, int kchunks, int skip, const Frags<PIN> &f) {
     f32x4 fa[2];
     float fb[2][4];
-    const int li = w.lane & 31, lh = w.lane >> 5;
-    const int a_off = (w.wm * 32 + li) * LW_BK, b_off = w.wn * 32 + li;
-    auto frag_load = [&](int buf, int slot, int kb) __attribute__((always_inline)) {
-      const float *as = smem_lw + slot * SLOT + a_off;
-      const float *bs = smem_lw + slot * SLOT + A_STAGE + b_off;
-      fa[buf] = *(const f32x4 *)(as + (((2 * kb + lh) ^ (li & 15)) << 2));
-#pragma unroll
-      for (int s = 0; s < 4; ++s) fb[buf][s] = bs[(8 * kb + 4 * lh + s) * BN];
-    };
-    const int kbw = w.wk * KB_PER_WAVE;
+    auto frag_load = [&](int buf, int slot, int q) __attribute__((always_inline)) { f.load(fa[buf], fb[buf], slot, q); };
+    const int kbw = f.kbw;
     auto chunk = [&](auto slot_c, auto rag_c, int first, bool has_next_rt) __attribute__((always_inline)) {
       constexpr int S = decltype(slot_c)::value, NS = (S + 1) % NSLOT;
       constexpr bool RAG = decltype(rag_c)::value != 0;
@@ -210,8 +288,8 @@
 #pragma unroll
       for (int q = 0; q < KB_PER_WAVE; ++q) {
         const int cur = q & 1, nxt = cur ^ 1;
-        if (q + 1 < KB_PER_WAVE) frag_load(nxt, S, kbw + q + 1);
-        else frag_load(nxt, NS, kbw);
+        if (q + 1 < KB_PER_WAVE) frag_load(nxt, S, q + 1);
+        else frag_load(nxt, NS, 0);
         __builtin_amdgcn_sched_barrier(0);
         if (!RAG || kedge_block_runs(kbw + q, first)) {
 #pragma unroll
@@ -233,7 +311,7 @@
     using R0 = std::integral_constant<int, 0>;
     using R1 = std::integral_constant<int, 1>;
 
-    frag_load(0, 0, kbw);
+    frag_load(0, 0, 0);
     int t = 0, c = 0;
     for (;;) {
       if (c + NSLOT < kchunks) {
@@ -261,30 +339,72 @@
     }
   }
 
-  static __device__ __forceinline__ void park_partials(const f32x16 &acc, const Wave &w) {
+  template <bool PIN> struct Tail {
+    unsigned park;
+    unsigned src[IPG];
+    unsigned off[IPG];
+    Wave w;
+    int ldc;
+  };
+  template <bool PIN = true> static __device__ __forceinline__ Tail<PIN> tail_setup(const Wave &w, int ldc) {
+    Tail<PIN> t = {0u, {}, {}, w, ldc};
+    if constexpr (PIN && WK > 1) {
+      t.park = lw_lds_addr(smem_lw + (w.wk * (WM * WN) + w.wmn) * 1024 + w.lane);
+      asm volatile("" : "+v"(t.park));
+#pragma unroll
+      for (int j = 0; j < IPG; ++j) {
+        const int q = piece_row(w, j);
+        const int r = (q & 3) + 4 * (q >> 3), lh2 = (q >> 2) & 1;
+        t.src[j] = lw_lds_addr(smem_lw + w.wmn * 1024 + r * 64 + lh2 * 32 + 4 * (w.lane & 7));
+        t.off[j] = piece_off(w, j, ldc);
+        asm volatile("" : "+v"(t.src[j]), "+v"(t.off[j]));
+      }
+    }
+    return t;
+  }
+  template <bool PIN> static __device__ __forceinline__ unsigned tail_off(const Tail<PIN> &t, int j) {
+    if constexpr (PIN) return t.off[j];
+    else return piece_off(t.w, j, t.ldc);
+  }
+  template <bool PIN> static __device__ __forceinline__ void park_partials(const f32x16 &acc, const Tail<PIN> &t) {
     __syncthreads();
-    float *dst = smem_lw + (w.wk * (WM * WN) + w.wmn) * 1024 + w.lane;
-#pragma unroll
-    for (int r = 0; r < 16; ++r) dst[r * 64] = acc[r];
+    if constexpr (PIN) {
+      lds_float_lw *dst = lw_lds_float(t.park);
+#pragma unroll
+      for (int r = 0; r < 16; ++r) dst[r * 64] = acc[r];
+    } else {
+      float *dst = smem_lw + (t.w.wk * (WM * WN) + t.w.wmn) * 1024 + t.w.lane;
+#pragma unroll
+      for (int r = 0; r < 16; ++r) dst[r * 64] = acc[r];
+    }
     __syncthreads();
   }
   static __device__ __forceinline__ int piece_row(const Wave &w, int j) { return 8 * (w.wk * IPG + j) + (w.lane >> 3); }
   static __device__ __forceinline__ unsigned piece_off(const Wave &w, int j, int ldc) {
     return (unsigned)(((w.wm * 32 + piece_row(w, j)) * ldc + w.wn * 32 + 4 * (w.lane & 7)) * 4);
   }
-  static __device__ __forceinline__ void sum_partials(f32x4 (&part)[IPG], const Wave &w) {
+  template <bool PIN> static __device__ __forceinline__ void sum_partials(f32x4 (&part)[IPG], const Tail<PIN> &t) {
 #pragma unroll
     for (int j = 0; j < IPG; ++j) {
-      const int q = piece_row(w, j);
-      const int r = (q & 3) + 4 * (q >> 3), lh2 = (q >> 2) & 1;
-      const float *src = smem_lw + w.wmn * 1024 + r * 64 + lh2 * 32 + 4 * (w.lane & 7);
-      f32x4 v = *(const f32x4 *)src;
-#pragma unroll
-      for (int g = 1; g < WK; ++g) v += *(const f32x4 *)(src + g * (WM * WN) * 1024);
-      part[j] = v;
-    }
-  }
-  static __device__ __forceinline__ void finish(const f32x4 (&part)[IPG], f32x4 bias4, int ep, __amdgpu_buffer_rsrc_t rsrcC, int ldc, bool ok, const Wave &w) {
+      if constexpr (PIN) {
+        const lds_f32x4_lw *src = lw_lds_f32x4(t.src[j]);
+        f32x4 v = *src;
+#pragma unroll
+        for (int g = 1; g < WK; ++g) v += src[g * (WM * WN) * 256];
+        part[j] = v;
+      } else {
+        const int q = piece_row(t.w, j);
+        const int r = (q & 3) + 4 * (q >> 3), lh2 = (q >> 2) & 1;
+        const float *src = smem_lw + t.w.wmn * 1024 + r * 64 + lh2 * 32 + 4 * (t.w.lane & 7);
+        f32x4 v = *(const f32x4 *)src;
+#pragma unroll
+        for (int g = 1; g < WK; ++g) v += *(const f32x4 *)(src + g * (WM * WN) * 1024);
+        part[j] = v;
+      }
+    }
+  }
+  template <bool PIN>
+  static __device__ __forceinline__ void finish(const f32x4 (&part)[IPG], f32x4 bias4, int ep, __amdgpu_buffer_rsrc_t rsrcC, bool ok, const Tail<PIN> &t) {
 #pragma unroll
     for (int j = 0; j < IPG; ++j) {
       f32x4 v = part[j] + bias4;
@@ -292,14 +412,15 @@
 #pragma unroll
         for (int e = 0; e < 4; ++e) v[e] = v[e] > 0.0f ? v[e] : 0.0f;
       }
-      if (ok) __builtin_amdgcn_raw_buffer_store_b128(__builtin_bit_cast(u32x4, v), rsrcC, piece_off(w, j, ldc), 0, LW_C_AUX);
+      if (ok) __builtin_amdgcn_raw_buffer_store_b128(__builtin_bit_cast(u32x4, v), rsrcC, tail_off(t, j), 0, LW_C_AUX);
     }
   }
   static __device__ __forceinline__ bool piece_owned(const Wave &w, int j, int own_r, int own_c) {
     return w.wm * 32 + piece_row(w, j) >= own_r && w.wn * 32 + 4 * (w.lane & 7) >= own_c;
   }
-  static __device__ __forceinline__ void finish_owned(const f32x4 (&part)[IPG], f32x4 bias4, int ep, __amdgpu_buffer_rsrc_t rsrcC, int ldc, int own_r, int own_c,
-                                                      const Wave &w) {
+  template <bool PIN>
+  static __device__ __forceinline__ void finish_owned(const f32x4 (&part)[IPG], f32x4 bias4, int ep, __amdgpu_buffer_rsrc_t rsrcC, int own_r, int own_c,
+                                                      const Wave &w, const Tail<PIN> &t) {
 #pragma unroll
     for (int j = 0; j < IPG; ++j) {
       f32x4 v = part[j] + bias4;
@@ -307,7 +428,7 @@
 #pragma unroll
         for (int e = 0; e < 4; ++e) v[e] = v[e] > 0.0f ? v[e] : 0.0f;
       }
-      if (piece_owned(w, j, own_r, own_c)) __builtin_amdgcn_raw_buffer_store_b128(__builtin_bit_cast(u32x4, v), rsrcC, piece_off(w, j, ldc), 0, LW_C_AUX);
+      if (piece_owned(w, j, own_r, own_c)) __builtin_amdgcn_raw_buffer_store_b128(__builtin_bit_cast(u32x4, v), rsrcC, tail_off(t, j), 0, LW_C_AUX);
     }
   }
 };
```
